# usnistgov/object-detection-yolov3

Hardware: AMD Instinct MI355X
Metric: images/sec (train fwd+bwd) bs=8 416x416 (higher is better)
Workload: dtype f32

## Files before the change

### include/yolo3hip.h

```cpp
#ifndef YOLO3HIP_H
#define YOLO3HIP_H

#include <math.h>
#include <stddef.h>
#include <stdint.h>

#ifdef __cplusplus
extern "C" {
#endif

#define Y3_OK 0
#define Y3_EINVAL (-1)
#define Y3_ELAUNCH (-2)

typedef void* y3_stream_t;

const char* y3_last_error(void);
int y3_debug_div(int x, int d);
int y3_version(void);

#define Y3_EPI_LRELU 1u
#define Y3_EPI_ACCUM 2u
#define Y3_CONV_X3 4u
int y3_x3_split_weights(const float* w, void* planes, int taps, int rows, int k_per_row, y3_stream_t stream);
// ... 92 lines not shown
int y3_conv2d_fwd_bf16_ws(const y3_tensor* src, const void* wt_t_bf16, const float* bias, int ksize, int stride,
                          const y3_tensor* dst, int dst_is_f32, unsigned flags, float alpha,
                          const float* scale, const float* shift, const y3_tensor* resid,
                          void* workspace, size_t workspace_bytes, y3_stream_t stream);
#define Y3_BF16_ROUTE_PP 1
#define Y3_BF16_ROUTE_C32 2
#define Y3_BF16_ROUTE_C64 3
#define Y3_BF16_ROUTE_RING 4
size_t y3_conv2d_fwd_bf16_plan(const y3_tensor* src, const void* wt_t_bf16, const float* bias, int ksize, int stride,
                               const y3_tensor* dst, int dst_is_f32, unsigned flags, float alpha,
                               const float* scale, const float* shift, const y3_tensor* resid,
                               void* workspace, size_t workspace_bytes, int* out12);
int y3_conv2d_first_bf16(const y3_tensor* src, const float* wt, const float* bias, const y3_tensor* dst,
                         unsigned flags, float alpha, const float* scale, const float* shift, y3_stream_t stream);
int y3_f32_to_bf16(const float* src, void* dst, size_t count, y3_stream_t stream);
int y3_upsample_sum2x_fwd_bf16(const y3_tensor* in, const y3_tensor* out, y3_stream_t stream);

int y3_copy(const y3_tensor* src, const y3_tensor* dst, y3_stream_t stream);
int y3_add_inplace(const y3_tensor* src, const y3_tensor* dst, y3_stream_t stream);
int y3_fill(float* ptr, size_t count, float value, y3_stream_t stream);
int y3_nchw_to_nhwc(const float* src, int n, int c, int h, int w, const y3_tensor* dst, y3_stream_t stream);
int y3_nhwc_to_nchw(const y3_tensor* src, float* dst, y3_stream_t stream);
int y3_colsum(const y3_tensor* src, float* out, y3_stream_t stream);

int y3_decode_fwd(const y3_tensor* fm, int nscales, const float* anchors_host, int num_anchors,
                  int num_classes, int img_h, int img_w, float* out, y3_stream_t stream);

int y3_loss_fwd_bwd(const y3_tensor* fm, const float* gt, const float* anchors_host, int num_anchors,
                    int num_classes, int img_h, int img_w, float global_batch,
                    float* loss4, const y3_tensor* dfm, void* workspace, y3_stream_t stream);
size_t y3_loss_workspace_bytes(void);

#define Y3_BOX_LOSS_MSE  0
#define Y3_BOX_LOSS_GIOU 1
#define Y3_BOX_LOSS_DIOU 2
#define Y3_BOX_LOSS_CIOU 3
int y3_loss_fwd_bwd_ex(const y3_tensor* fm, const float* gt, const float* anchors_host, int num_anchors,
                       int num_classes, int img_h, int img_w, float global_batch, int box_loss, float box_weight,
                       float* loss4, const y3_tensor* dfm, void* workspace, y3_stream_t stream);

#define Y3_TRUTH_CHUNK 256
int y3_truth_boxes(const float* gt, int n, long long cells_anchors, int d, float* boxes, int* counts, int cap,
                   y3_stream_t stream);
size_t y3_loss_truth_workspace_bytes(int n);
int y3_loss_fwd_bwd_truth(const y3_tensor* fm, const float* gt, const float* anchors_host, int num_anchors,
                          int num_classes, int img_h, int img_w, float global_batch, int box_loss, float box_weight,
                          const float* truth_boxes, const int* truth_counts, int truth_cap, float ignore_thresh,
                          float* loss4, float* ignored, const y3_tensor* dfm, void* workspace, y3_stream_t stream);

int y3_loss_fwd_bwd_focal(const y3_tensor* fm, const float* gt, const float* anchors_host, int num_anchors,
                          int num_classes, int img_h, int img_w, float global_batch, int box_loss, float box_weight,
                          const float* truth_boxes, const int* truth_counts, int truth_cap, float ignore_thresh,
                          float* loss4, float* ignored, const y3_tensor* dfm, void* workspace, float gamma_obj,
                          float alpha_obj, float gamma_cls, float alpha_cls, float label_smoothing, y3_stream_t stream);

int y3_adam_step(float* param, const float* grad, float* m, float* v, size_t count,
                 const float* lr_t_dev, float beta1, float beta2, float eps, y3_stream_t stream);

int y3_adam_step_ema(float* param, const float* grad, float* m, float* v, size_t count,
                     const float* lr_t_dev, float beta1, float beta2, float eps,
                     float* ema_param, const float* moving, float* ema_moving, size_t moving_count,
                     const float* omd_dev, y3_stream_t stream);

#define Y3_GRAD_CLIP_OFF ((double)INFINITY)
size_t y3_grad_norm_workspace_bytes(size_t count);
int y3_grad_accumulate(float* acc, const float* grad, size_t count, const int* first_dev, void* workspace,
                       y3_stream_t stream);
int y3_grad_sumsq(const float* grad, size_t count, void* workspace, y3_stream_t stream);
int y3_grad_clip_scale(const void* workspace, size_t count, int accumulate_steps, double clip_norm, float* norm_dev,
                       float* scale_dev, y3_stream_t stream);
int y3_adam_step_scaled(float* param, const float* grad, float* m, float* v, size_t count,
                        const float* lr_t_dev, float beta1, float beta2, float eps, const float* scale_dev,
                        y3_stream_t stream);
int y3_adam_step_ema_scaled(float* param, const float* grad, float* m, float* v, size_t count,
                            const float* lr_t_dev, float beta1, float beta2, float eps,
                            float* ema_param, const float* moving, float* ema_moving, size_t moving_count,
                            const float* omd_dev, const float* scale_dev, y3_stream_t stream);
// ... 194 lines not shown
```

### object-detection-yolov3_amd/csrc/detect.hip

```cpp
#include <float.h>
#include <stdlib.h>

#include "common.h"

#define Y3_MAX_ANCHORS 16
#define Y3_MAX_SCALES 4

__device__ __forceinline__ float sigmoidf_(float x) { return 1.f / (1.f + expf(-x)); }

struct DecodeArgs {
    const float* fm[Y3_MAX_SCALES];
    int ld[Y3_MAX_SCALES], gh[Y3_MAX_SCALES], gw[Y3_MAX_SCALES], start[Y3_MAX_SCALES + 1];
    float sx[Y3_MAX_SCALES], sy[Y3_MAX_SCALES];
    float aw[Y3_MAX_ANCHORS], ah[Y3_MAX_ANCHORS];
    int nscales, A, K, N, nb;
    float* out;
};

__global__ void decode_kernel(const DecodeArgs p) {
    const long long total = (long long)p.N * p.nb;
    const long long stride = (long long)gridDim.x * blockDim.x;
    const int D = 5 + p.K;
    for (long long i = (long long)blockIdx.x * blockDim.x + threadIdx.x; i < total; i += stride) {
        const int n = (int)(i / p.nb);
// ... 137 lines not shown
            const float alpha = v / ((1.0f - iou) + v + 1e-7f);
            X = X - alpha * v;
            const float a_at = alpha * (2.0f * k * da);
            const float q = bw * bw + bh * bh;
            a_bw = a_at * (bh / q);
            a_bh = -(a_at * (bw / q));
        }
    }
    const float a_inter = 1.0f / U - a_U;
    a_bw += a_U * bh;
    a_bh += a_U * bw;
    const float a_ixr = ixr >= 0.f ? a_inter * iy : 0.f, a_iyr = iyr >= 0.f ? a_inter * ix : 0.f;
    const float a_px1 = px1 < gx1 ? a_ixr : (px1 > gx1 ? a_cw : 0.5f * (a_ixr + a_cw));
    const float a_px0 = px0 > gx0 ? -a_ixr : (px0 < gx0 ? -a_cw : -0.5f * (a_ixr + a_cw));
    const float a_py1 = py1 < gy1 ? a_iyr : (py1 > gy1 ? a_ch : 0.5f * (a_iyr + a_ch));
    const float a_py0 = py0 > gy0 ? -a_iyr : (py0 < gy0 ? -a_ch : -0.5f * (a_iyr + a_ch));
    gb[0] = -(a_bx + (a_px0 + a_px1));
    gb[1] = -(a_by + (a_py0 + a_py1));
    gb[2] = -(a_bw + (a_px1 - a_px0) / 2.0f);
    gb[3] = -(a_bh + (a_py1 - a_py0) / 2.0f);
    return 1.0f - X;
}

template <int BOX, bool TRUTH, bool FOCAL>
__global__ __launch_bounds__(256) void loss_kernel(const LossArgs p) {
    constexpr int NP = TRUTH ? 5 : 4;
    __shared__ float sm[NP][256];
    __shared__ float4 tb[TRUTH ? Y3_TRUTH_CHUNK : 1];
    const int D = 5 + p.K;
    const long long total = TRUTH ? (long long)p.G_h * p.G_w * p.A : (long long)p.N * p.G_h * p.G_w * p.A;
    const long long first = TRUTH ? (long long)blockIdx.y * total : 0;
    const long long stride = (long long)gridDim.x * blockDim.x;
    float l_xy = 0.f, l_wh = 0.f, l_obj = 0.f, l_cls = 0.f, l_ign = 0.f;
    int cnt = 0;
    const float* tbox = nullptr;
    if (TRUTH) {
        cnt = p.truth_counts[blockIdx.y];
        cnt = cnt < 0 ? 0 : (cnt > p.truth_cap ? p.truth_cap : cnt);
        tbox = p.truth_boxes + (long long)blockIdx.y * p.truth_cap * 4;
        if (cnt <= Y3_TRUTH_CHUNK) {
            if ((int)threadIdx.x < cnt) {
                const float* b = tbox + (long long)threadIdx.x * 4;
                tb[threadIdx.x] = make_float4(b[0], b[1], b[2], b[3]);
            }
            __syncthreads();
        }
    }
    for (long long j = (long long)blockIdx.x * blockDim.x + threadIdx.x; TRUTH ? j - threadIdx.x < total : j < total; j += stride) {
        const bool active = !TRUTH || j < total;
        const long long i = TRUTH ? first + (active ? j : total - 1) : j;
        const int a = (int)(i % p.A);
        const long long cell = i / p.A;
        const int gx = (int)(cell % p.G_w);
        const int gy = (int)((cell / p.G_w) % p.G_h);
        const float* t = p.fm + cell * p.fm_ld + a * D;
        const float* g = p.gt + i * D;
        float* d = p.dfm + cell * p.dfm_ld + a * D;
        const float aw = p.aw[a], ah = p.ah[a];
        const float offx = (float)gx, offy = (float)gy;
        const float sgx = sigmoidf_(t[0]), sgy = sigmoidf_(t[1]);
        const float bx = (sgx + offx) * p.sx, by = (sgy + offy) * p.sy;
        const float ew = expf(t[2]), eh = expf(t[3]);
        const float bw = ew * aw, bh = eh * ah;
        const float gm = g[4];

        float best = -INFINITY;
        if (!TRUTH) {
            for (int q = 0; q < p.A; ++q) {
                if (!p.present[q]) continue;
                const float tw = p.aw[q], th = p.ah[q];
                const float ix = fmaxf(fminf(bx + bw / 2.0f, tw / 2.0f) - fmaxf(bx - bw / 2.0f, -tw / 2.0f), 0.f);
// ... 90 lines not shown
                gb[0] = w * (gb[0] * (p.sx * (sgx * (1.f - sgx)))) * p.gscale;
                gb[1] = w * (gb[1] * (p.sy * (sgy * (1.f - sgy)))) * p.gscale;
                gb[2] = w * (gb[2] * bw) * p.gscale;
                gb[3] = w * (gb[3] * bh) * p.gscale;
            }
            d[0] = gb[0];
            d[1] = gb[1];
            d[2] = gb[2];
            d[3] = gb[3];
        }
    }
    sm[0][threadIdx.x] = l_xy;
    sm[1][threadIdx.x] = l_wh;
    sm[2][threadIdx.x] = l_obj;
    sm[3][threadIdx.x] = l_cls;
    if (TRUTH) sm[NP - 1][threadIdx.x] = l_ign;
    __syncthreads();
    for (int o = 128; o > 0; o >>= 1) {
        if (threadIdx.x < o)
#pragma unroll
            for (int j = 0; j < NP; ++j) sm[j][threadIdx.x] += sm[j][threadIdx.x + o];
        __syncthreads();
    }
    if (!TRUTH) {
        if (threadIdx.x < 4) p.partials[blockIdx.x * 4 + threadIdx.x] = sm[threadIdx.x][0] * p.inv_b;
    } else if (threadIdx.x < NP) {
        p.partials[((long long)blockIdx.y * gridDim.x + blockIdx.x) * NP + threadIdx.x] = sm[threadIdx.x][0] * (threadIdx.x < 4 ? p.inv_b : 1.f);
    }
}

__global__ void loss_clear_kernel(int* present) {
    if (threadIdx.x < Y3_MAX_ANCHORS) present[threadIdx.x] = 0;
}
__global__ void loss_finalize_kernel(const float* partials, int nblocks, float* loss4) {
    if (threadIdx.x < 4) {
        float s = 0.f;
        for (int b = 0; b < nblocks; ++b) s += partials[b * 4 + threadIdx.x];
        loss4[threadIdx.x] += s;
    }
}

__global__ __launch_bounds__(256) void loss_finalize_truth_kernel(const float* partials, int n, int bpi, float* loss4, float* ignored) {
    __shared__ float slots[32][8];
    const int j = threadIdx.x & 7, slot = threadIdx.x >> 3;
    float s = 0.f;
    if (j < 5)
        for (int img = slot; img < n; img += 32)
            for (int b = 0; b < bpi; ++b) s += partials[((long long)img * bpi + b) * 5 + j];
    slots[slot][j] = s;
    __syncthreads();
    if (threadIdx.x < 5) {
        float t = 0.f;
        for (int q = 0; q < 32; ++q) t += slots[q][threadIdx.x];
        if (threadIdx.x < 4)
            loss4[threadIdx.x] += t;
        else if (ignored)
            *ignored += t;
    }
}

#define Y3_LOSS_BLOCKS 64
extern "C" size_t y3_loss_workspace_bytes(void) { return (Y3_MAX_ANCHORS + Y3_LOSS_BLOCKS * 4) * sizeof(float); }

#define Y3_LOSS_TRUTH_BLOCKS 16
extern "C" size_t y3_loss_truth_workspace_bytes(int n) {
    if (n < 1) return 0;
    return (size_t)n * Y3_LOSS_TRUTH_BLOCKS * 5 * sizeof(float);
}

struct LossTruth {
    const float* boxes;
    const int* counts;
    int cap;
    float thresh;
    float* ignored;
};

struct LossFocal {
    float gamma_obj, alpha_obj, gamma_cls, alpha_cls, label_smoothing;
};

template <bool TRUTH, bool FOCAL>
static void loss_kernel_launch_kind(int box_loss, dim3 grid, hipStream_t st, const LossArgs& p) {
    if (box_loss == Y3_BOX_LOSS_MSE)
        hipLaunchKernelGGL((loss_kernel<Y3_BOX_LOSS_MSE, TRUTH, FOCAL>), grid, dim3(256), 0, st, p);
    else if (box_loss == Y3_BOX_LOSS_GIOU)
        hipLaunchKernelGGL((loss_kernel<Y3_BOX_LOSS_GIOU, TRUTH, FOCAL>), grid, dim3(256), 0, st, p);
    else if (box_loss == Y3_BOX_LOSS_DIOU)
        hipLaunchKernelGGL((loss_kernel<Y3_BOX_LOSS_DIOU, TRUTH, FOCAL>), grid, dim3(256), 0, st, p);
    else
        hipLaunchKernelGGL((loss_kernel<Y3_BOX_LOSS_CIOU, TRUTH, FOCAL>), grid, dim3(256), 0, st, p);
}

template <bool TRUTH>
static void loss_kernel_launch(int box_loss, bool focal, dim3 grid, hipStream_t st, const LossArgs& p) {
    if (focal)
        loss_kernel_launch_kind<TRUTH, true>(box_loss, grid, st, p);
    else
        loss_kernel_launch_kind<TRUTH, false>(box_loss, grid, st, p);
}

static int loss_launch(const y3_tensor* fm, const float* gt, const float* anchors_host, int num_anchors, int num_classes, int img_h, int img_w,
                       float global_batch, int box_loss, float box_weight, const LossTruth* truth, const LossFocal* focal, float* loss4,
                       const y3_tensor* dfm, void* workspace, y3_stream_t stream) {
    bool use_focal = false;
    if (focal) {
        const float go = focal->gamma_obj, ao = focal->alpha_obj, gc = focal->gamma_cls, ac = focal->alpha_cls, ls = focal->label_smoothing;
        Y3_CHECK_ARG(go >= 0.f && go <= FLT_MAX && gc >= 0.f && gc <= FLT_MAX, "loss_fwd_bwd_focal: gamma must be finite and >= 0 (got %g, %g)",
                     (double)go, (double)gc);
        Y3_CHECK_ARG((ao == 0.f || (ao > 0.f && ao < 1.f)) && (ac == 0.f || (ac > 0.f && ac < 1.f)),
                     "loss_fwd_bwd_focal: alpha must be 0 (no balancing factor) or in (0, 1) (got %g, %g)", (double)ao, (double)ac);
        Y3_CHECK_ARG(ls >= 0.f && ls < 1.f, "loss_fwd_bwd_focal: label_smoothing must be in [0, 1) (got %g)", (double)ls);
        use_focal = !(go == 0.f && ao == 0.f && gc == 0.f && ac == 0.f && ls == 0.f);
    }
    if (truth) {
        Y3_CHECK_ARG(truth->thresh > 0.f && truth->thresh <= 1.f, "loss_fwd_bwd_truth: ignore_thresh must be finite and in (0, 1] (got %g)",
                     (double)truth->thresh);
        Y3_CHECK_ARG(truth->cap >= 1, "loss_fwd_bwd_truth: truth_cap %d (at least 1)", truth->cap);
        Y3_CHECK_ARG(truth->boxes && truth->counts, "loss_fwd_bwd_truth: null pointer (truth_boxes, truth_counts)");
    }
    Y3_CHECK_ARG(box_loss >= Y3_BOX_LOSS_MSE && box_loss <= Y3_BOX_LOSS_CIOU, "loss_fwd_bwd: unknown box_loss %d", box_loss);
    Y3_CHECK_ARG(box_weight > 0.f && box_weight <= FLT_MAX, "loss_fwd_bwd: box_weight must be finite and > 0 (got %g)", (double)box_weight);
    Y3_CHECK_ARG(box_loss != Y3_BOX_LOSS_MSE || box_weight == 1.f, "loss_fwd_bwd: box_weight %g needs an IoU box_loss (mse takes 1)",
                 (double)box_weight);
    Y3_CHECK_ARG(fm && fm->ptr && dfm && dfm->ptr && gt && anchors_host && loss4 && workspace, "loss_fwd_bwd: null pointer");
    Y3_CHECK_ARG(num_anchors >= 1 && num_anchors <= Y3_MAX_ANCHORS && num_classes >= 1, "loss_fwd_bwd: anchors/classes");
    const int D = num_anchors * (5 + num_classes);
    Y3_CHECK_ARG(fm->c == D && dfm->c == D && fm->ld >= D && dfm->ld >= D && dfm->n == fm->n && dfm->h == fm->h && dfm->w == fm->w, "loss_fwd_bwd: geometry");
    hipStream_t st = (hipStream_t)stream;
    LossArgs p = {};
    p.fm = fm->ptr;
    p.gt = gt;
    p.dfm = dfm->ptr;
    p.fm_ld = fm->ld;
    p.dfm_ld = dfm->ld;
    p.N = fm->n;
    p.G_h = fm->h;
    p.G_w = fm->w;
    p.A = num_anchors;
    p.K = num_classes;
    p.sx = (float)(img_h / fm->h);
    p.sy = (float)(img_w / fm->w);
    for (int a = 0; a < num_anchors; ++a) {
        p.aw[a] = anchors_host[2 * a];
        p.ah[a] = anchors_host[2 * a + 1];
    }
    p.inv_b = 1.f / (float)fm->n;
    p.gscale = 1.f / ((float)fm->n * global_batch);
    p.box_weight = box_weight;
    if (use_focal) {
        p.gamma_obj = focal->gamma_obj;
        p.alpha_obj = focal->alpha_obj;
        p.gamma_cls = focal->gamma_cls;
        p.alpha_cls = focal->alpha_cls;
        p.label_smoothing = focal->label_smoothing;
    }
    if (truth) {
        Y3_CHECK_ARG(fm->n <= 65535, "loss_fwd_bwd_truth: batch %d (at most 65535 images per call)", fm->n);
        const long long per_image = (long long)p.G_h * p.G_w * p.A;
        int bpi = (int)((per_image + 255) / 256);
        if (bpi > Y3_LOSS_TRUTH_BLOCKS) bpi = Y3_LOSS_TRUTH_BLOCKS;
        p.partials = (float*)workspace;
        p.truth_boxes = truth->boxes;
        p.truth_counts = truth->counts;
        p.truth_cap = truth->cap;
        p.ignore_thresh = truth->thresh;
        loss_kernel_launch<true>(box_loss, use_focal, dim3(bpi, p.N), st, p);
        Y3_CHECK_LAUNCH("loss (truth mask)");
        hipLaunchKernelGGL(loss_finalize_truth_kernel, dim3(1), dim3(256), 0, st, (const float*)p.partials, p.N, bpi, loss4, truth->ignored);
        Y3_CHECK_LAUNCH("loss_finalize (truth mask)");
        return Y3_OK;
    }
    p.present = (int*)workspace;
    p.partials = (float*)workspace + Y3_MAX_ANCHORS;
    hipLaunchKernelGGL(loss_clear_kernel, dim3(1), dim3(64), 0, st, p.present);
    Y3_CHECK_LAUNCH("loss_clear");
    const long long total = (long long)p.N * p.G_h * p.G_w * p.A;
    int pb = (int)((total + 255) / 256);
    if (pb > 256) pb = 256;
// ... 20 lines not shown
    return loss_launch(fm, gt, anchors_host, num_anchors, num_classes, img_h, img_w, global_batch, box_loss, box_weight, nullptr, nullptr, loss4,
                       dfm, workspace, stream);
}

extern "C" int y3_loss_fwd_bwd_truth(const y3_tensor* fm, const float* gt, const float* anchors_host, int num_anchors, int num_classes,
                                     int img_h, int img_w, float global_batch, int box_loss, float box_weight, const float* truth_boxes,
                                     const int* truth_counts, int truth_cap, float ignore_thresh, float* loss4, float* ignored,
                                     const y3_tensor* dfm, void* workspace, y3_stream_t stream) {
    const LossTruth truth = {truth_boxes, truth_counts, truth_cap, ignore_thresh, ignored};
    return loss_launch(fm, gt, anchors_host, num_anchors, num_classes, img_h, img_w, global_batch, box_loss, box_weight, &truth, nullptr, loss4,
                       dfm, workspace, stream);
}

extern "C" int y3_loss_fwd_bwd_focal(const y3_tensor* fm, const float* gt, const float* anchors_host, int num_anchors, int num_classes,
                                     int img_h, int img_w, float global_batch, int box_loss, float box_weight, const float* truth_boxes,
                                     const int* truth_counts, int truth_cap, float ignore_thresh, float* loss4, float* ignored,
                                     const y3_tensor* dfm, void* workspace, float gamma_obj, float alpha_obj, float gamma_cls,
                                     float alpha_cls, float label_smoothing, y3_stream_t stream) {
    const LossTruth truth = {truth_boxes, truth_counts, truth_cap, ignore_thresh, ignored};
    const LossFocal focal = {gamma_obj, alpha_obj, gamma_cls, alpha_cls, label_smoothing};
    const bool reference_mask = !truth_boxes && !truth_counts;
    return loss_launch(fm, gt, anchors_host, num_anchors, num_classes, img_h, img_w, global_batch, box_loss, box_weight,
                       reference_mask ? nullptr : &truth, &focal, loss4, dfm, workspace, stream);
}

__global__ __launch_bounds__(256) void truth_boxes_kernel(const float* __restrict__ gt, int ca, int d, float* __restrict__ boxes,
                                                         int* __restrict__ counts, int cap) {
    __shared__ int wave_cnt[4];
    const int tid = threadIdx.x, lane = tid & 63, wave = tid >> 6;
    const float* g = gt + (long long)blockIdx.x * ca * d;
    float* out = boxes + (long long)blockIdx.x * cap * 4;
    int base = 0;
    for (int r0 = 0; r0 < ca; r0 += 256) {
        const int r = r0 + tid;
        const float* row = g + (long long)(r < ca ? r : 0) * d;
        const bool keep = r < ca && row[4] != 0.f;
        const unsigned long long bal = __ballot(keep);
        if (lane == 0) wave_cnt[wave] = __popcll(bal);
        __syncthreads();
        int off = base;
        for (int w = 0; w < wave; ++w) off += wave_cnt[w];
        const int pos = off + __popcll(bal & ((1ull << lane) - 1ull));
        if (keep && pos < cap) {
            float* dst = out + (long long)pos * 4;
            dst[0] = row[0];
            dst[1] = row[1];
// ... 874 lines not shown
```

### object-detection-yolov3_amd/csrc/pointwise.hip

```cpp
#include "common.h"

static int check_view(const y3_tensor* t, const char* name) {
    Y3_CHECK_ARG(t && t->ptr, "%s: null tensor", name);
    Y3_CHECK_ARG(t->n > 0 && t->h > 0 && t->w > 0 && t->c > 0 && t->ld >= t->c, "%s: bad dims", name);
    return 0;
}
static int check_view4(const y3_tensor* t, const char* name) {
    if (int e = check_view(t, name)) return e;
    Y3_CHECK_ARG((t->c & 3) == 0 && (t->ld & 3) == 0 && ((uintptr_t)t->ptr & 15) == 0, "%s: needs c, ld multiples of 4 and 16-byte alignment", name);
    return 0;
}
static inline long long pixels(const y3_tensor* t) { return (long long)t->n * t->h * t->w; }
static inline bool same_geom(const y3_tensor* a, const y3_tensor* b) { return a->n == b->n && a->h == b->h && a->w == b->w && a->c == b->c; }

__global__ __launch_bounds__(1024) void bn_stats_finalize_kernel(const float* __restrict__ stats, int tiles, int C, double inv_count,
                                                                 double bessel, const float* __restrict__ gamma,
                                                                 const float* __restrict__ beta, float eps, float momentum,
                                                                 float* moving_mean, float* moving_var, float* save_mean,
                                                                 float* save_rstd, float* scale, float* shift) {
    __shared__ double sm[1024][4];
    const int which = threadIdx.x & 1, lane = threadIdx.x >> 1;
    const int c0 = blockIdx.x * 4;
    double acc[4] = {0.0, 0.0, 0.0, 0.0};
    for (int t = lane; t < tiles; t += 512) {
// ... 875 lines not shown
    Y3_CHECK_LAUNCH("nchw_to_nhwc");
    return Y3_OK;
}
__global__ void nhwc_to_nchw_kernel(const float* __restrict__ src, int s_ld, int C, long long hw, float* __restrict__ dst, long long total) {
    const long long stride = (long long)gridDim.x * blockDim.x;
    for (long long i = (long long)blockIdx.x * blockDim.x + threadIdx.x; i < total; i += stride) {
        const long long r = i % hw;
        const long long nc = i / hw;
        const long long n = nc / C;
        const int c = (int)(nc - n * C);
        dst[i] = src[(n * hw + r) * s_ld + c];
    }
}
extern "C" int y3_nhwc_to_nchw(const y3_tensor* src, float* dst, y3_stream_t stream) {
    if (int e = check_view(src, "nhwc_to_nchw src")) return e;
    Y3_CHECK_ARG(dst, "nhwc_to_nchw: null dst");
    const long long total = pixels(src) * src->c;
    hipLaunchKernelGGL(nhwc_to_nchw_kernel, dim3(stream_blocks(total, 256)), dim3(256), 0, (hipStream_t)stream, src->ptr, src->ld, src->c,
                       (long long)src->h * src->w, dst, total);
    Y3_CHECK_LAUNCH("nhwc_to_nchw");
    return Y3_OK;
}

__global__ __launch_bounds__(1024) void colsum_kernel(const float* __restrict__ src, int ld, int C, long long npix, float* __restrict__ out) {
    __shared__ double sm[1024];
    const int c = blockIdx.x;
    double s = 0.0;
    for (long long r = threadIdx.x; r < npix; r += 1024) s += (double)src[r * ld + c];
    sm[threadIdx.x] = s;
    __syncthreads();
    for (int o = 512; o > 0; o >>= 1) {
        if (threadIdx.x < o) sm[threadIdx.x] += sm[threadIdx.x + o];
        __syncthreads();
    }
    if (threadIdx.x == 0) out[c] = (float)sm[0];
}
extern "C" int y3_colsum(const y3_tensor* src, float* out, y3_stream_t stream) {
    if (int e = check_view(src, "colsum src")) return e;
    Y3_CHECK_ARG(out && src->c <= 65535, "colsum: bad args");
    hipLaunchKernelGGL(colsum_kernel, dim3(src->c), dim3(1024), 0, (hipStream_t)stream, src->ptr, src->ld, src->c, pixels(src), out);
    Y3_CHECK_LAUNCH("colsum");
    return Y3_OK;
}

#define Y3_ZS_BLOCKS 128
__global__ __launch_bounds__(256) void zscore_partial_kernel(const float* __restrict__ in, size_t count, double* __restrict__ ws) {
    __shared__ double sm[2][256];
    const int img = blockIdx.y;
    const float* src = in + (size_t)img * count;
    double s = 0.0, q = 0.0;
    for (size_t i = (size_t)blockIdx.x * 256 + threadIdx.x; i < count; i += (size_t)Y3_ZS_BLOCKS * 256) {
        const double v = (double)src[i];
        s += v;
        q += v * v;
    }
    sm[0][threadIdx.x] = s;
    sm[1][threadIdx.x] = q;
    __syncthreads();
    for (int o = 128; o > 0; o >>= 1) {
        if (threadIdx.x < o) {
            sm[0][threadIdx.x] += sm[0][threadIdx.x + o];
            sm[1][threadIdx.x] += sm[1][threadIdx.x + o];
        }
        __syncthreads();
// ... 204 lines not shown
```

### object-detection-yolov3_amd/yolo3/_hip.py

```python
import ctypes as C
import os

import torch

_HERE = os.path.dirname(os.path.abspath(__file__))
LIB_PATH = os.environ.get('Y3_LIB') or os.path.join(_HERE, '_lib', 'libyolo3hip.so')


class HipLibraryMissing(ImportError):
    pass


class HipError(RuntimeError):
    pass


if not os.path.exists(LIB_PATH):
    raise HipLibraryMissing(
        'libyolo3hip.so not found at %s: build it with `make -C object-detection-yolov3_amd/csrc` '
        '(hipcc --offload-arch=gfx950).  There is no CPU fallback.' % LIB_PATH)

lib = C.CDLL(LIB_PATH)


# ... 60 lines not shown
    'y3_conv2d_fwd_bf16': (i32, [TP, vp, fp, i32, i32, TP, i32, u32, f32, fp, fp, TP, vp]),
    'y3_conv2d_fwd_bf16_ws': (i32, [TP, vp, fp, i32, i32, TP, i32, u32, f32, fp, fp, TP, vp, sz, vp]),
    'y3_conv2d_fwd_bf16_workspace': (sz, [i32, i32, i32, i32]),
    'y3_conv2d_fwd_bf16_plan': (sz, [TP, vp, fp, i32, i32, TP, i32, u32, f32, fp, fp, TP, vp, sz, ip]),
    'y3_f32_to_bf16': (i32, [fp, vp, sz, vp]),
    'y3_conv2d_first_bf16': (i32, [TP, fp, fp, TP, u32, f32, fp, fp, vp]),
    'y3_tile_gather': (i32, [vp, i32, i32, i32, i32, ip, i32, i32, i32, fp, vp]),
    'y3_tile_gather_zscore_nhwc': (i32, [vp, i32, i32, i32, i32, ip, i32, i32, i32, fp, i32, vp, vp]),
    'y3_upsample_sum2x_fwd_bf16': (i32, [TP, TP, vp]),
    'y3_add_inplace': (i32, [TP, TP, vp]),
    'y3_fill': (i32, [fp, sz, f32, vp]),
    'y3_nchw_to_nhwc': (i32, [fp, i32, i32, i32, i32, TP, vp]),
    'y3_nhwc_to_nchw': (i32, [TP, fp, vp]),
    'y3_colsum': (i32, [TP, fp, vp]),
    'y3_decode_fwd': (i32, [TP, i32, C.POINTER(C.c_float), i32, i32, i32, i32, fp, vp]),
    'y3_loss_fwd_bwd': (i32, [TP, fp, C.POINTER(C.c_float), i32, i32, i32, i32, f32, fp, TP, vp, vp]),
    'y3_loss_fwd_bwd_ex': (i32, [TP, fp, C.POINTER(C.c_float), i32, i32, i32, i32, f32, i32, f32, fp, TP, vp, vp]),
    'y3_loss_workspace_bytes': (sz, []),
    'y3_truth_boxes': (i32, [fp, i32, C.c_longlong, i32, fp, ip, i32, vp]),
    'y3_loss_truth_workspace_bytes': (sz, [i32]),
    'y3_loss_fwd_bwd_truth': (i32, [TP, fp, C.POINTER(C.c_float), i32, i32, i32, i32, f32, i32, f32, fp, ip, i32, f32, fp, fp, TP, vp, vp]),
    'y3_loss_fwd_bwd_focal': (i32, [TP, fp, C.POINTER(C.c_float), i32, i32, i32, i32, f32, i32, f32, fp, ip, i32, f32, fp, fp, TP, vp, f32, f32, f32,
                                    f32, f32, vp]),
    'y3_adam_step': (i32, [fp, fp, fp, fp, sz, fp, f32, f32, f32, vp]),
    'y3_adam_step_ema': (i32, [fp, fp, fp, fp, sz, fp, f32, f32, f32, fp, fp, fp, sz, fp, vp]),
    'y3_grad_norm_workspace_bytes': (sz, [sz]),
    'y3_grad_accumulate': (i32, [fp, fp, sz, ip, vp, vp]),
    'y3_grad_sumsq': (i32, [fp, sz, vp, vp]),
    'y3_grad_clip_scale': (i32, [vp, sz, i32, C.c_double, fp, fp, vp]),
    'y3_adam_step_scaled': (i32, [fp, fp, fp, fp, sz, fp, f32, f32, f32, fp, vp]),
    'y3_adam_step_ema_scaled': (i32, [fp, fp, fp, fp, sz, fp, f32, f32, f32, fp, fp, fp, sz, fp, fp, vp]),
    'y3_optim_step': (i32, [C.POINTER(OptimDesc), vp]),
    'y3_nms_per_class': (i32, [fp, i32, i32, i32, f32, f32, f32, f32, f32, ip, ip, fp, i32, vp, sz, vp]),
    'y3_nms_workspace_bytes': (sz, [i32, i32, i32]),
    'y3_nms_single_class': (i32, [fp, i32, f32, ip, ip, fp, vp, sz, vp]),
    'y3_nms_per_class_ex': (i32, [fp, i32, i32, i32, i32, f32, f32, f32, f32, f32, f32, ip, ip, fp, i32, vp, sz, vp]),
    'y3_nms_workspace_bytes_ex': (sz, [i32, i32, i32, i32]),
    'y3_nms_labelled': (i32, [fp, i32, i32, i32, f32, f32, f32, ip, ip, fp, i32, vp, sz, vp]),
    'y3_tile_merge': (i32, [fp, i32, i32, i32, i32, ip, ip, fp, i32, ip, i32, i32, i32, i32, i32, f32, fp, i32, ip, vp, sz, vp]),
    'y3_tile_merge_workspace_bytes': (sz, [i32, i32]),
    'y3_tta_views_nhwc': (i32, [fp, i32, i32, i32, i32, C.POINTER(C.c_int), i32, TP, vp]),
    'y3_tta_unmap': (i32, [fp, i32, i32, i32, C.POINTER(C.c_int), i32, i32, i32, vp]),
    'y3_box_vote': (i32, [fp, i32, i32, i32, ip, ip, fp, i32, f32, f32, f32, f32, f32, i32, i32, i32, fp, vp, sz, vp]),
    'y3_box_vote_workspace_bytes': (sz, [i32, i32, i32]),
    'y3_filter_small_boxes': (i32, [fp, i32, i32, f32, ip, ip, vp]),
    'y3_compute_iou': (i32, [fp, fp, i32, i32, fp, vp]),
# ... 69 lines not shown
```

### object-detection-yolov3_amd/yolo3/model.py

```python
import collections
import contextlib
import ctypes
import functools
import math
import os
import warnings

import numpy as np
import torch

from . import _hip
from . import letterbox
from . import streams
from ._hip import lib, check, view, int_array, EPI_LRELU, EPI_ACCUM, CONV_X3, BF16_NO_PATCH

BN_EPS = 1e-3
BN_MOMENTUM = 0.99
LRELU_ALPHA = 0.2
BF16_PATCH_MIN_BYTES = 300e6
ALIGN = 64


def ema_one_minus_decay(ema_decay, ema_warmup, t):
    d = float(ema_decay) * (1.0 - math.exp(-float(t) / float(ema_warmup)))
# ... 599 lines not shown
            ws = self._at(self.loss_ws, si * ws_floats)
            if focal is not None:
                truth = mdl.ignore_mask == 'truth'
                self.loss_calls.append((lib.y3_loss_fwd_bwd_focal, (f.v, g.data_ptr(), mdl.anchors_c, A, K, H, W, float(mdl.global_batch_size),
                                                                    BOX_LOSSES.index(mdl.box_loss), mdl.box_loss_weight,
                                                                    self.truth_boxes.data_ptr() if truth else None,
                                                                    self.truth_counts.data_ptr() if truth else None,
                                                                    cap if truth else 1, mdl.ignore_thresh, self.loss4.data_ptr(),
                                                                    self.ignored.data_ptr() if truth else None, f.grad.v, ws) + focal))
            elif mdl.ignore_mask == 'truth':
                self.loss_calls.append((lib.y3_loss_fwd_bwd_truth, (f.v, g.data_ptr(), mdl.anchors_c, A, K, H, W, float(mdl.global_batch_size),
                                                                    BOX_LOSSES.index(mdl.box_loss), mdl.box_loss_weight,
                                                                    self.truth_boxes.data_ptr(), self.truth_counts.data_ptr(), cap,
                                                                    mdl.ignore_thresh, self.loss4.data_ptr(), self.ignored.data_ptr(),
                                                                    f.grad.v, ws)))
            elif mdl.box_loss == 'mse':
                self.loss_calls.append((lib.y3_loss_fwd_bwd, (f.v, g.data_ptr(), mdl.anchors_c, A, K, H, W, float(mdl.global_batch_size),
                                                              self.loss4.data_ptr(), f.grad.v, ws)))
            else:
                self.loss_calls.append((lib.y3_loss_fwd_bwd_ex, (f.v, g.data_ptr(), mdl.anchors_c, A, K, H, W, float(mdl.global_batch_size),
                                                                 BOX_LOSSES.index(mdl.box_loss), mdl.box_loss_weight,
                                                                 self.loss4.data_ptr(), f.grad.v, ws)))
            f.gw = True
        if tr:
            self._build_backward()
        self._bind_conv_workspace()

    def _grad_of(self, t):
        if t.grad is None:
            if t.parent is not None:
                self._grad_of(t.parent)
                return t.grad
            t.grad = self._new(t.n, t.h, t.w, t.c, t.ld)
            for ch in t.children:
                ch.grad = _T(t.grad.buf, ch.n, ch.h, ch.w, ch.c, ch.ld, ch.off)
        return t.grad

    def _kernel_grad(self, fn, *args):
        args += (self.wg_ws.data_ptr(), self.wg_ws_bytes)
        if self.side is None:
            self._emit(self.bwd, fn, *args)
            return None
        self.events += [torch.cuda.Event(), torch.cuda.Event()]
        e_go, e_wg = len(self.events) - 2, len(self.events) - 1
        self.bwd.append(('record', e_go))
        self.keep.append(args)
        self.bwd.append(('side_call', (fn, args, e_go, e_wg)))
        return e_wg

# ... 33 lines not shown
                    first_consumer.setdefault(id(ch), op)
        for op in self.ops:
            if op[0] != 'conv_layer' or mdl.freeze_bn:
                continue
            a, y = op[3], op[4]
            cons = first_consumer.get(id(y))
            if cons is None or cons[0] != 'conv_layer' or cons[2] is not y or y.children or y is self.x0:
                continue
            csp = specs[cons[1]]
            tiles = int(lib.y3_conv2d_dgrad_bn_tiles_x(cons[3].v, csp.k, csp.s, y.v, cons[-1].dgrad))
            if tiles <= 0:
                continue
            part = torch.empty(tiles * 6 * y.c, dtype=torch.float32, device=mdl.device)
            epi_of[id(cons)] = (a, part, tiles)
            epi_for[id(op)] = (part, tiles)
        self.epilogue_stats_layers = len(epi_for)
        two = (not mdl.use_graph) and os.environ.get('Y3_WGRAD_STREAM', '1') != '0'
        self.side = streams.reserve(mdl.device)[0] if two else None
        self.events = []
        dz_bufs = [self.dz, torch.empty_like(self.dz)] if two else [self.dz]
        dz_busy = [None, None]
        head_wg = None
        nconv = 0
        for op in reversed(self.ops):
            kind = op[0]
            if kind == 'head':
                _, i, src, fm, _ = op
                sp = specs[i]
                dfm = fm.grad
                self._emit(self.bwd, lib.y3_colsum, dfm.v, gptr(sp.b_off))
                head_wg = self._kernel_grad(lib.y3_conv2d_wgrad, src.v, dfm.v, 1, 1, gptr(sp.w_off))
                if not src.no_grad:
                    ds = self._grad_of(src)
                    self._conv_call(self.bwd, lib.y3_conv2d_dgrad, dfm.v, self._at(mdl.params_t, sp.w_off), 1, 1, ds.v, EPI_ACCUM if src.gw else 0)
                    src.mark_written()
                self.bwd.append(('layer_done', i))
            elif kind == 'upsample':
                _, src, dst = op
                assert dst.gw and not src.gw
                ds = self._grad_of(src)
                self._emit(self.bwd, lib.y3_upsample_sum2x_bwd, dst.grad.v, ds.v)
                src.mark_written()
            elif kind == 'spp':
                _, src, cat, pools = op
                assert cat.gw and src.gw
                self._emit(self.bwd, lib.y3_spp_bwd, src.v, pools.grad.v, src.grad.v, 1)
            else:
                _, i, src, a, y, resid, x3 = op
                smean, srstd, coef = x3.bn
                sp = specs[i]
                assert y.gw, 'gradient of layer %d output never produced' % i
                dy = y.grad
                dr = None
# ... 72 lines not shown
                    self.side.wait_event(self.events[e_wait])
                    rc = f2(*a2, self.side.cuda_stream)
                    if rc != 0:
                        check(rc, f2.__name__)
                    self.events[e_done].record(self.side)
                    pending.append(e_done)
                continue
            rc = fn(*args, stream)
            if rc != 0:
                check(rc, fn.__name__)

    def run_forward(self, stream, skip_input=False):
        self._run(self.fwd[1:] if skip_input else self.fwd, stream)

    def run_decode(self, stream):
        fn, args = self.decode_call
        check(fn(*args, stream), 'y3_decode_fwd')

    def run_inference(self, stream, skip_input=False):
        self.run_forward(stream, skip_input)
        self.run_decode(stream)

    def run_loss(self, stream):
        check(lib.y3_fill(self.loss4.data_ptr(), 4, 0.0, stream), 'y3_fill')
        if self.truth_call is not None:
            check(lib.y3_fill(self.ignored.data_ptr(), 1, 0.0, stream), 'y3_fill')
            fn, args = self.truth_call
            check(fn(*args, stream), 'y3_truth_boxes')
        for fn, args in self.loss_calls:
            check(fn(*args, stream), fn.__name__)

    def run_backward(self, stream, dist=None):
        self._run(self.bwd, stream, dist)


class _CallableModel:

    def __init__(self, yolo, feature_maps):
        self._y = yolo
        self._fm = feature_maps

    supports_slots = True

    def __call__(self, batch, training=False, slot=0):
        if self._fm:
            return self._y.feature_maps(batch, training=training)
# ... 795 lines not shown
```

Before: 568.9.

## Batch per-scale loss and head bias colsum into grouped single launches

Replaces the per-scale YOLO loss launches (fill, present-mask, loss kernel, reduce) with two grouped kernels covering all scales. The loss kernel does its final reduction in the last block through an atomic ticket, and that block also clears the present flags. The three head bias-gradient column sums are merged into one grouped launch. The aim is to cut kernel-launch and host overhead on small tail kernels, at the cost of a last-block atomic reduction scheme with relaxed memory ordering.

```diff
diff --git a/include/yolo3hip.h b/include/yolo3hip.h
--- a/include/yolo3hip.h
+++ b/include/yolo3hip.h
@@ -138,6 +138,7 @@
 int y3_nchw_to_nhwc(const float* src, int n, int c, int h, int w, const y3_tensor* dst, y3_stream_t stream);
 int y3_nhwc_to_nchw(const y3_tensor* src, float* dst, y3_stream_t stream);
 int y3_colsum(const y3_tensor* src, float* out, y3_stream_t stream);
+int y3_colsum_group(const y3_tensor* src, float* const* out, int count, y3_stream_t stream);
 
 int y3_decode_fwd(const y3_tensor* fm, int nscales, const float* anchors_host, int num_anchors,
                   int num_classes, int img_h, int img_w, float* out, y3_stream_t stream);
@@ -169,6 +170,14 @@
                           const float* truth_boxes, const int* truth_counts, int truth_cap, float ignore_thresh,
                           float* loss4, float* ignored, const y3_tensor* dfm, void* workspace, float gamma_obj,
                           float alpha_obj, float gamma_cls, float alpha_cls, float label_smoothing, y3_stream_t stream);
+
+size_t y3_loss_group_workspace_bytes(int nscales);
+int y3_loss_present_group(const float* const* gt, const y3_tensor* fm, int nscales, int num_anchors, int num_classes,
+                          void* workspace, size_t workspace_bytes, y3_stream_t stream);
+int y3_loss_fwd_bwd_group(const y3_tensor* fm, const float* const* gt, int nscales, const float* anchors_host,
+                          int num_anchors, int num_classes, int img_h, int img_w, float global_batch, int box_loss,
+                          float box_weight, const float* focal_host, float* loss4, const y3_tensor* dfm, void* workspace,
+                          size_t workspace_bytes, y3_stream_t stream);
 
 int y3_adam_step(float* param, const float* grad, float* m, float* v, size_t count,
                  const float* lr_t_dev, float beta1, float beta2, float eps, y3_stream_t stream);
diff --git a/object-detection-yolov3_amd/csrc/detect.hip b/object-detection-yolov3_amd/csrc/detect.hip
--- a/object-detection-yolov3_amd/csrc/detect.hip
+++ b/object-detection-yolov3_amd/csrc/detect.hip
@@ -183,15 +183,15 @@
     return 1.0f - X;
 }
 
-template <int BOX, bool TRUTH, bool FOCAL>
-__global__ __launch_bounds__(256) void loss_kernel(const LossArgs p) {
+template <int BOX, bool TRUTH, bool FOCAL, bool GROUP>
+__device__ __forceinline__ void loss_block(const LossArgs& p, const int bx, const int nbx) {
     constexpr int NP = TRUTH ? 5 : 4;
     __shared__ float sm[NP][256];
     __shared__ float4 tb[TRUTH ? Y3_TRUTH_CHUNK : 1];
     const int D = 5 + p.K;
     const long long total = TRUTH ? (long long)p.G_h * p.G_w * p.A : (long long)p.N * p.G_h * p.G_w * p.A;
     const long long first = TRUTH ? (long long)blockIdx.y * total : 0;
-    const long long stride = (long long)gridDim.x * blockDim.x;
+    const long long stride = (long long)nbx * blockDim.x;
     float l_xy = 0.f, l_wh = 0.f, l_obj = 0.f, l_cls = 0.f, l_ign = 0.f;
     int cnt = 0;
     const float* tbox = nullptr;
@@ -207,7 +207,7 @@
             __syncthreads();
         }
     }
-    for (long long j = (long long)blockIdx.x * blockDim.x + threadIdx.x; TRUTH ? j - threadIdx.x < total : j < total; j += stride) {
+    for (long long j = (long long)bx * blockDim.x + threadIdx.x; TRUTH ? j - threadIdx.x < total : j < total; j += stride) {
         const bool active = !TRUTH || j < total;
         const long long i = TRUTH ? first + (active ? j : total - 1) : j;
         const int a = (int)(i % p.A);
@@ -344,11 +344,19 @@
             for (int j = 0; j < NP; ++j) sm[j][threadIdx.x] += sm[j][threadIdx.x + o];
         __syncthreads();
     }
-    if (!TRUTH) {
-        if (threadIdx.x < 4) p.partials[blockIdx.x * 4 + threadIdx.x] = sm[threadIdx.x][0] * p.inv_b;
+    if (GROUP) {
+        if (threadIdx.x < 4)
+            __hip_atomic_store(p.partials + bx * 4 + threadIdx.x, sm[threadIdx.x][0] * p.inv_b, __ATOMIC_RELAXED, __HIP_MEMORY_SCOPE_AGENT);
+    } else if (!TRUTH) {
+        if (threadIdx.x < 4) p.partials[bx * 4 + threadIdx.x] = sm[threadIdx.x][0] * p.inv_b;
     } else if (threadIdx.x < NP) {
-        p.partials[((long long)blockIdx.y * gridDim.x + blockIdx.x) * NP + threadIdx.x] = sm[threadIdx.x][0] * (threadIdx.x < 4 ? p.inv_b : 1.f);
-    }
+        p.partials[((long long)blockIdx.y * nbx + bx) * NP + threadIdx.x] = sm[threadIdx.x][0] * (threadIdx.x < 4 ? p.inv_b : 1.f);
+    }
+}
+
+template <int BOX, bool TRUTH, bool FOCAL>
+__global__ __launch_bounds__(256) void loss_kernel(const LossArgs p) {
+    loss_block<BOX, TRUTH, FOCAL, false>(p, blockIdx.x, gridDim.x);
 }
 
 __global__ void loss_clear_kernel(int* present) {
@@ -384,6 +392,74 @@
 #define Y3_LOSS_BLOCKS 64
 extern "C" size_t y3_loss_workspace_bytes(void) { return (Y3_MAX_ANCHORS + Y3_LOSS_BLOCKS * 4) * sizeof(float); }
 
+#define Y3_LOSS_GROUP_MAX 3
+#define Y3_LOSS_GROUP_HEAD 16
+extern "C" size_t y3_loss_group_workspace_bytes(int nscales) {
+    if (nscales < 1 || nscales > Y3_LOSS_GROUP_MAX) return 0;
+    return (Y3_LOSS_GROUP_HEAD + (size_t)nscales * (Y3_MAX_ANCHORS + Y3_LOSS_BLOCKS * 4)) * sizeof(float);
+}
+
+struct PresentGroupArgs {
+    const float* gt[Y3_LOSS_GROUP_MAX];
+    long long total[Y3_LOSS_GROUP_MAX];
+    int* present[Y3_LOSS_GROUP_MAX];
+    int first[Y3_LOSS_GROUP_MAX + 1];
+    int nscales, A, D;
+};
+
+__global__ __launch_bounds__(256) void loss_present_group_kernel(const PresentGroupArgs g) {
+    int s = 0;
+    while (s + 1 < g.nscales && (int)blockIdx.x >= g.first[s + 1]) ++s;
+    const long long stride = (long long)(g.first[s + 1] - g.first[s]) * blockDim.x;
+    const float* __restrict__ gt = g.gt[s];
+    const long long total = g.total[s];
+    for (long long i = (long long)((int)blockIdx.x - g.first[s]) * blockDim.x + threadIdx.x; i < total; i += stride)
+        if (gt[i * g.D + 4] != 0.f) atomicOr(&g.present[s][i % g.A], 1);
+}
+
+struct LossGroupArgs {
+    LossArgs s[Y3_LOSS_GROUP_MAX];
+    int first[Y3_LOSS_GROUP_MAX + 1];
+    int nscales;
+    int* ticket;
+    float* loss4;
+};
+
+template <int BOX, bool FOCAL>
+__global__ __launch_bounds__(256) void loss_group_kernel(const LossGroupArgs g) {
+    __shared__ int last_flag;
+    int s = 0;
+    while (s + 1 < g.nscales && (int)blockIdx.x >= g.first[s + 1]) ++s;
+    loss_block<BOX, false, FOCAL, true>(g.s[s], (int)blockIdx.x - g.first[s], g.first[s + 1] - g.first[s]);
+    asm volatile("s_waitcnt vmcnt(0)" ::: "memory");
+    __syncthreads();
+    if (threadIdx.x == 0) {
+        const int old = __hip_atomic_fetch_add(g.ticket, 1, __ATOMIC_RELAXED, __HIP_MEMORY_SCOPE_AGENT);
+        const int last = old == (int)gridDim.x - 1;
+        if (last) __hip_atomic_store(g.ticket, 0, __ATOMIC_RELAXED, __HIP_MEMORY_SCOPE_AGENT);
+        last_flag = last;
+    }
+    __syncthreads();
+    if (last_flag == 0) return;
+    __shared__ float fin[Y3_LOSS_GROUP_MAX][Y3_LOSS_BLOCKS * 4];
+    for (int k = 0; k < g.nscales; ++k)
+        if ((int)threadIdx.x < (g.first[k + 1] - g.first[k]) * 4)
+            fin[k][threadIdx.x] = __hip_atomic_load(g.s[k].partials + threadIdx.x, __ATOMIC_RELAXED, __HIP_MEMORY_SCOPE_AGENT);
+    __syncthreads();
+    if (threadIdx.x < 4) {
+        float t = 0.f;
+        for (int k = 0; k < g.nscales; ++k) {
+            const int nb = g.first[k + 1] - g.first[k];
+            float sk = 0.f;
+            for (int b = 0; b < nb; ++b) sk += fin[k][b * 4 + threadIdx.x];
+            t += sk;
+        }
+        g.loss4[threadIdx.x] = t;
+    } else if (threadIdx.x >= 64 && threadIdx.x < 64 + Y3_MAX_ANCHORS) {
+        for (int k = 0; k < g.nscales; ++k) __hip_atomic_store(g.s[k].present + (threadIdx.x - 64), 0, __ATOMIC_RELAXED, __HIP_MEMORY_SCOPE_AGENT);
+    }
+}
+
 #define Y3_LOSS_TRUTH_BLOCKS 16
 extern "C" size_t y3_loss_truth_workspace_bytes(int n) {
     if (n < 1) return 0;
@@ -422,10 +498,10 @@
         loss_kernel_launch_kind<TRUTH, false>(box_loss, grid, st, p);
 }
 
-static int loss_launch(const y3_tensor* fm, const float* gt, const float* anchors_host, int num_anchors, int num_classes, int img_h, int img_w,
-                       float global_batch, int box_loss, float box_weight, const LossTruth* truth, const LossFocal* focal, float* loss4,
-                       const y3_tensor* dfm, void* workspace, y3_stream_t stream) {
-    bool use_focal = false;
+static int loss_prepare(const y3_tensor* fm, const float* gt, const float* anchors_host, int num_anchors, int num_classes, int img_h, int img_w,
+                        float global_batch, int box_loss, float box_weight, const LossTruth* truth, const LossFocal* focal, float* loss4,
+                        const y3_tensor* dfm, void* workspace, LossArgs& p, bool& use_focal) {
+    use_focal = false;
     if (focal) {
         const float go = focal->gamma_obj, ao = focal->alpha_obj, gc = focal->gamma_cls, ac = focal->alpha_cls, ls = focal->label_smoothing;
         Y3_CHECK_ARG(go >= 0.f && go <= FLT_MAX && gc >= 0.f && gc <= FLT_MAX, "loss_fwd_bwd_focal: gamma must be finite and >= 0 (got %g, %g)",
@@ -449,8 +525,7 @@
     Y3_CHECK_ARG(num_anchors >= 1 && num_anchors <= Y3_MAX_ANCHORS && num_classes >= 1, "loss_fwd_bwd: anchors/classes");
     const int D = num_anchors * (5 + num_classes);
     Y3_CHECK_ARG(fm->c == D && dfm->c == D && fm->ld >= D && dfm->ld >= D && dfm->n == fm->n && dfm->h == fm->h && dfm->w == fm->w, "loss_fwd_bwd: geometry");
-    hipStream_t st = (hipStream_t)stream;
-    LossArgs p = {};
+    p = LossArgs{};
     p.fm = fm->ptr;
     p.gt = gt;
     p.dfm = dfm->ptr;
@@ -477,6 +552,18 @@
         p.alpha_cls = focal->alpha_cls;
         p.label_smoothing = focal->label_smoothing;
     }
+    return Y3_OK;
+}
+
+static int loss_launch(const y3_tensor* fm, const float* gt, const float* anchors_host, int num_anchors, int num_classes, int img_h, int img_w,
+                       float global_batch, int box_loss, float box_weight, const LossTruth* truth, const LossFocal* focal, float* loss4,
+                       const y3_tensor* dfm, void* workspace, y3_stream_t stream) {
+    LossArgs p;
+    bool use_focal;
+    if (int e = loss_prepare(fm, gt, anchors_host, num_anchors, num_classes, img_h, img_w, global_batch, box_loss, box_weight, truth, focal, loss4,
+                             dfm, workspace, p, use_focal))
+        return e;
+    hipStream_t st = (hipStream_t)stream;
     if (truth) {
         Y3_CHECK_ARG(fm->n <= 65535, "loss_fwd_bwd_truth: batch %d (at most 65535 images per call)", fm->n);
         const long long per_image = (long long)p.G_h * p.G_w * p.A;
@@ -543,6 +630,83 @@
     const bool reference_mask = !truth_boxes && !truth_counts;
     return loss_launch(fm, gt, anchors_host, num_anchors, num_classes, img_h, img_w, global_batch, box_loss, box_weight,
                        reference_mask ? nullptr : &truth, &focal, loss4, dfm, workspace, stream);
+}
+
+static int loss_group_blocks(const y3_tensor* fm, int num_anchors, int cap) {
+    const long long total = (long long)fm->n * fm->h * fm->w * num_anchors;
+    const long long blocks = (total + 255) / 256;
+    return blocks > cap ? cap : (int)blocks;
+}
+
+extern "C" int y3_loss_present_group(const float* const* gt, const y3_tensor* fm, int nscales, int num_anchors, int num_classes, void* workspace,
+                                     size_t workspace_bytes, y3_stream_t stream) {
+    Y3_CHECK_ARG(nscales >= 1 && nscales <= Y3_LOSS_GROUP_MAX, "loss_present_group: %d scales (1 to %d)", nscales, Y3_LOSS_GROUP_MAX);
+    Y3_CHECK_ARG(gt && fm && workspace, "loss_present_group: null pointer");
+    Y3_CHECK_ARG(num_anchors >= 1 && num_anchors <= Y3_MAX_ANCHORS && num_classes >= 1, "loss_present_group: anchors/classes");
+    Y3_CHECK_ARG(workspace_bytes >= y3_loss_group_workspace_bytes(nscales), "loss_present_group: workspace of %zu bytes (%zu needed)",
+                 workspace_bytes, y3_loss_group_workspace_bytes(nscales));
+    PresentGroupArgs g = {};
+    g.nscales = nscales;
+    g.A = num_anchors;
+    g.D = 5 + num_classes;
+    int* flags = (int*)workspace + Y3_LOSS_GROUP_HEAD;
+    for (int s = 0; s < nscales; ++s) {
+        Y3_CHECK_ARG(gt[s] && fm[s].n >= 1 && fm[s].h >= 1 && fm[s].w >= 1, "loss_present_group: scale %d: null labels or empty geometry", s);
+        Y3_CHECK_ARG(fm[s].n == fm[0].n, "loss_present_group: scale %d has batch %d, scale 0 has %d", s, fm[s].n, fm[0].n);
+        g.gt[s] = gt[s];
+        g.total[s] = (long long)fm[s].n * fm[s].h * fm[s].w * num_anchors;
+        g.present[s] = flags + s * Y3_MAX_ANCHORS;
+        g.first[s + 1] = g.first[s] + loss_group_blocks(&fm[s], num_anchors, 256);
+    }
+    hipLaunchKernelGGL(loss_present_group_kernel, dim3(g.first[nscales]), dim3(256), 0, (hipStream_t)stream, g);
+    Y3_CHECK_LAUNCH("loss_present_group");
+    return Y3_OK;
+}
+
+template <bool FOCAL>
+static void loss_group_launch_kind(int box_loss, dim3 grid, hipStream_t st, const LossGroupArgs& g) {
+    if (box_loss == Y3_BOX_LOSS_MSE)
+        hipLaunchKernelGGL((loss_group_kernel<Y3_BOX_LOSS_MSE, FOCAL>), grid, dim3(256), 0, st, g);
+    else if (box_loss == Y3_BOX_LOSS_GIOU)
+        hipLaunchKernelGGL((loss_group_kernel<Y3_BOX_LOSS_GIOU, FOCAL>), grid, dim3(256), 0, st, g);
+    else if (box_loss == Y3_BOX_LOSS_DIOU)
+        hipLaunchKernelGGL((loss_group_kernel<Y3_BOX_LOSS_DIOU, FOCAL>), grid, dim3(256), 0, st, g);
+    else
+        hipLaunchKernelGGL((loss_group_kernel<Y3_BOX_LOSS_CIOU, FOCAL>), grid, dim3(256), 0, st, g);
+}
+
+extern "C" int y3_loss_fwd_bwd_group(const y3_tensor* fm, const float* const* gt, int nscales, const float* anchors_host, int num_anchors,
+                                     int num_classes, int img_h, int img_w, float global_batch, int box_loss, float box_weight,
+                                     const float* focal_host, float* loss4, const y3_tensor* dfm, void* workspace, size_t workspace_bytes,
+                                     y3_stream_t stream) {
+    Y3_CHECK_ARG(nscales >= 1 && nscales <= Y3_LOSS_GROUP_MAX, "loss_fwd_bwd_group: %d scales (1 to %d)", nscales, Y3_LOSS_GROUP_MAX);
+    Y3_CHECK_ARG(fm && gt && dfm && workspace, "loss_fwd_bwd_group: null pointer");
+    Y3_CHECK_ARG(workspace_bytes >= y3_loss_group_workspace_bytes(nscales), "loss_fwd_bwd_group: workspace of %zu bytes (%zu needed)",
+                 workspace_bytes, y3_loss_group_workspace_bytes(nscales));
+    LossFocal focal = {};
+    if (focal_host) focal = LossFocal{focal_host[0], focal_host[1], focal_host[2], focal_host[3], focal_host[4]};
+    LossGroupArgs g = {};
+    g.nscales = nscales;
+    g.ticket = (int*)workspace;
+    g.loss4 = loss4;
+    int* flags = (int*)workspace + Y3_LOSS_GROUP_HEAD;
+    float* partials = (float*)(flags + nscales * Y3_MAX_ANCHORS);
+    bool use_focal = false;
+    for (int s = 0; s < nscales; ++s) {
+        if (int e = loss_prepare(&fm[s], gt[s], anchors_host, num_anchors, num_classes, img_h, img_w, global_batch, box_loss, box_weight, nullptr,
+                                 focal_host ? &focal : nullptr, loss4, &dfm[s], workspace, g.s[s], use_focal))
+            return e;
+        Y3_CHECK_ARG(fm[s].n == fm[0].n, "loss_fwd_bwd_group: scale %d has batch %d, scale 0 has %d", s, fm[s].n, fm[0].n);
+        g.s[s].present = flags + s * Y3_MAX_ANCHORS;
+        g.s[s].partials = partials + s * (Y3_LOSS_BLOCKS * 4);
+        g.first[s + 1] = g.first[s] + loss_group_blocks(&fm[s], num_anchors, Y3_LOSS_BLOCKS);
+    }
+    if (use_focal)
+        loss_group_launch_kind<true>(box_loss, dim3(g.first[nscales]), (hipStream_t)stream, g);
+    else
+        loss_group_launch_kind<false>(box_loss, dim3(g.first[nscales]), (hipStream_t)stream, g);
+    Y3_CHECK_LAUNCH("loss_group");
+    return Y3_OK;
 }
 
 __global__ __launch_bounds__(256) void truth_boxes_kernel(const float* __restrict__ gt, int ca, int d, float* __restrict__ boxes,
diff --git a/object-detection-yolov3_amd/csrc/pointwise.hip b/object-detection-yolov3_amd/csrc/pointwise.hip
--- a/object-detection-yolov3_amd/csrc/pointwise.hip
+++ b/object-detection-yolov3_amd/csrc/pointwise.hip
@@ -921,9 +921,8 @@
     return Y3_OK;
 }
 
-__global__ __launch_bounds__(1024) void colsum_kernel(const float* __restrict__ src, int ld, int C, long long npix, float* __restrict__ out) {
+__device__ __forceinline__ void colsum_block(const float* __restrict__ src, int ld, int c, long long npix, float* __restrict__ out) {
     __shared__ double sm[1024];
-    const int c = blockIdx.x;
     double s = 0.0;
     for (long long r = threadIdx.x; r < npix; r += 1024) s += (double)src[r * ld + c];
     sm[threadIdx.x] = s;
@@ -933,12 +932,48 @@
         __syncthreads();
     }
     if (threadIdx.x == 0) out[c] = (float)sm[0];
+}
+__global__ __launch_bounds__(1024) void colsum_kernel(const float* __restrict__ src, int ld, int C, long long npix, float* __restrict__ out) {
+    colsum_block(src, ld, blockIdx.x, npix, out);
 }
 extern "C" int y3_colsum(const y3_tensor* src, float* out, y3_stream_t stream) {
     if (int e = check_view(src, "colsum src")) return e;
     Y3_CHECK_ARG(out && src->c <= 65535, "colsum: bad args");
     hipLaunchKernelGGL(colsum_kernel, dim3(src->c), dim3(1024), 0, (hipStream_t)stream, src->ptr, src->ld, src->c, pixels(src), out);
     Y3_CHECK_LAUNCH("colsum");
+    return Y3_OK;
+}
+
+#define Y3_COLSUM_GROUP_MAX 3
+struct ColsumGroupArgs {
+    const float* src[Y3_COLSUM_GROUP_MAX];
+    float* out[Y3_COLSUM_GROUP_MAX];
+    long long npix[Y3_COLSUM_GROUP_MAX];
+    int ld[Y3_COLSUM_GROUP_MAX];
+    int first[Y3_COLSUM_GROUP_MAX + 1];
+    int count;
+};
+__global__ __launch_bounds__(1024) void colsum_group_kernel(const ColsumGroupArgs g) {
+    int k = 0;
+    while (k + 1 < g.count && (int)blockIdx.x >= g.first[k + 1]) ++k;
+    colsum_block(g.src[k], g.ld[k], (int)blockIdx.x - g.first[k], g.npix[k], g.out[k]);
+}
+extern "C" int y3_colsum_group(const y3_tensor* src, float* const* out, int count, y3_stream_t stream) {
+    Y3_CHECK_ARG(count >= 1 && count <= Y3_COLSUM_GROUP_MAX, "colsum_group: %d tensors (1 to %d)", count, Y3_COLSUM_GROUP_MAX);
+    Y3_CHECK_ARG(src && out, "colsum_group: null pointer");
+    ColsumGroupArgs g = {};
+    g.count = count;
+    for (int k = 0; k < count; ++k) {
+        if (int e = check_view(&src[k], "colsum_group src")) return e;
+        Y3_CHECK_ARG(out[k] && src[k].c <= 65535, "colsum_group: bad args (tensor %d)", k);
+        g.src[k] = src[k].ptr;
+        g.out[k] = out[k];
+        g.npix[k] = pixels(&src[k]);
+        g.ld[k] = src[k].ld;
+        g.first[k + 1] = g.first[k] + src[k].c;
+    }
+    hipLaunchKernelGGL(colsum_group_kernel, dim3(g.first[count]), dim3(1024), 0, (hipStream_t)stream, g);
+    Y3_CHECK_LAUNCH("colsum_group");
     return Y3_OK;
 }
 
diff --git a/object-detection-yolov3_amd/yolo3/_hip.py b/object-detection-yolov3_amd/yolo3/_hip.py
--- a/object-detection-yolov3_amd/yolo3/_hip.py
+++ b/object-detection-yolov3_amd/yolo3/_hip.py
@@ -106,6 +106,11 @@
     'y3_loss_fwd_bwd_truth': (i32, [TP, fp, C.POINTER(C.c_float), i32, i32, i32, i32, f32, i32, f32, fp, ip, i32, f32, fp, fp, TP, vp, vp]),
     'y3_loss_fwd_bwd_focal': (i32, [TP, fp, C.POINTER(C.c_float), i32, i32, i32, i32, f32, i32, f32, fp, ip, i32, f32, fp, fp, TP, vp, f32, f32, f32,
                                     f32, f32, vp]),
+    'y3_loss_group_workspace_bytes': (sz, [i32]),
+    'y3_loss_present_group': (i32, [C.POINTER(C.c_void_p), TP, i32, i32, i32, vp, sz, vp]),
+    'y3_loss_fwd_bwd_group': (i32, [TP, C.POINTER(C.c_void_p), i32, C.POINTER(C.c_float), i32, i32, i32, i32, f32, i32, f32,
+                                    C.POINTER(C.c_float), fp, TP, vp, sz, vp]),
+    'y3_colsum_group': (i32, [TP, C.POINTER(C.c_void_p), i32, vp]),
     'y3_adam_step': (i32, [fp, fp, fp, fp, sz, fp, f32, f32, f32, vp]),
     'y3_adam_step_ema': (i32, [fp, fp, fp, fp, sz, fp, f32, f32, f32, fp, fp, fp, sz, fp, vp]),
     'y3_grad_norm_workspace_bytes': (sz, [sz]),
diff --git a/object-detection-yolov3_amd/yolo3/model.py b/object-detection-yolov3_amd/yolo3/model.py
--- a/object-detection-yolov3_amd/yolo3/model.py
+++ b/object-detection-yolov3_amd/yolo3/model.py
@@ -645,9 +645,34 @@
                                                                  BOX_LOSSES.index(mdl.box_loss), mdl.box_loss_weight,
                                                                  self.loss4.data_ptr(), f.grad.v, ws)))
             f.gw = True
+        self.loss_group = self._group_loss_calls()
         if tr:
             self._build_backward()
         self._bind_conv_workspace()
+
+    def _group_loss_calls(self):
+        per = []
+        for fn, a in self.loss_calls:
+            if fn is lib.y3_loss_fwd_bwd:
+                per.append(a[:8] + (0, 1.0, None) + a[8:])
+            elif fn is lib.y3_loss_fwd_bwd_ex:
+                per.append(a[:10] + (None,) + a[10:])
+            elif fn is lib.y3_loss_fwd_bwd_focal and a[10] is None and a[11] is None:
+                per.append(a[:10] + (_hip.float_array(a[18:23]), a[14], a[16], a[17]))
+            else:
+                return None
+        n = len(per)
+        shared = per[0][2:10] + (per[0][11],)
+        assert all(p[2:10] + (p[11],) == shared for p in per) and all(list(p[10] or ()) == list(per[0][10] or ()) for p in per)
+        fms = (_hip.Tensor * n)(*[p[0] for p in per])
+        dfms = (_hip.Tensor * n)(*[p[12] for p in per])
+        gts = (ctypes.c_void_p * n)(*[p[1] for p in per])
+        nbytes = int(lib.y3_loss_group_workspace_bytes(n))
+        self.loss_group_ws = torch.zeros(nbytes // 4, dtype=torch.float32, device=self.model.device)
+        ws = self.loss_group_ws.data_ptr()
+        anchors, A, K, H, W, gb, box, bw = per[0][2:10]
+        return [(lib.y3_loss_present_group, (gts, fms, n, A, K, ws, nbytes)),
+                (lib.y3_loss_fwd_bwd_group, (fms, gts, n, anchors, A, K, H, W, gb, box, bw, per[0][10], per[0][11], dfms, ws, nbytes))]
 
     def _grad_of(self, t):
         if t.grad is None:
@@ -727,13 +752,17 @@
         dz_busy = [None, None]
         head_wg = None
         nconv = 0
+        heads = [op for op in reversed(self.ops) if op[0] == 'head']
+        if heads:
+            srcs = (_hip.Tensor * len(heads))(*[op[3].grad.v for op in heads])
+            outs = (ctypes.c_void_p * len(heads))(*[gptr(specs[op[1]].b_off) for op in heads])
+            self._emit(self.bwd, lib.y3_colsum_group, srcs, outs, len(heads))
         for op in reversed(self.ops):
             kind = op[0]
             if kind == 'head':
                 _, i, src, fm, _ = op
                 sp = specs[i]
                 dfm = fm.grad
-                self._emit(self.bwd, lib.y3_colsum, dfm.v, gptr(sp.b_off))
                 head_wg = self._kernel_grad(lib.y3_conv2d_wgrad, src.v, dfm.v, 1, 1, gptr(sp.w_off))
                 if not src.no_grad:
                     ds = self._grad_of(src)
@@ -852,6 +881,10 @@
         self.run_decode(stream)
 
     def run_loss(self, stream):
+        if self.loss_group is not None:
+            for fn, args in self.loss_group:
+                check(fn(*args, stream), fn.__name__)
+            return
         check(lib.y3_fill(self.loss4.data_ptr(), 4, 0.0, stream), 'y3_fill')
         if self.truth_call is not None:
             check(lib.y3_fill(self.ignored.data_ptr(), 1, 0.0, stream), 'y3_fill')
```

Result: no change. 571.4, median of 3 (+0.4%).
